# Atif-Anwer/SHMGAN

Hardware: AMD Instinct MI355X
Metric: images/sec (gen+disc train_step) (higher is better)
Workload: dtype f32; 1 GPU; SHMGAN train_step 256x256 5-view, batch 8/GPU, filter_size 64, fp32 (BASELINE configs[1]); global_batch=8, image_size=256, parallelism=dp1, losses_finite=True

## Files before the change

include/shmgan_hip.h:

```cpp
#ifndef SHMGAN_HIP_H
#define SHMGAN_HIP_H

#include <stddef.h>

#ifdef __cplusplus
extern "C" {
#endif

#define SHM_OK 0
#define SHM_E_SHAPE (-1)
#define SHM_E_DTYPE (-2)
#define SHM_E_WORKSPACE (-3)
#define SHM_E_HIP (-4)

#define SHM_F32 0
#define SHM_BF16 1
#define SHM_BF16_GF32 2

int shm_version(void);
const char* shm_last_error(void);
const char* shm_last_kernel(void);

#define SHM_TG_AUTO 0
#define SHM_TG_HALO128 1
#define SHM_TG_HALO64 2
#define SHM_TG_DMA_128x128 3
#define SHM_TG_DMA_64x128 4
#define SHM_TG_DMA_128x64 5
#define SHM_TG_DMA_256x64 6
#define SHM_TG_DMA_256x128 7
#define SHM_TG_HALO128_PH8 8
#define SHM_TG_DMA_128x128_BK32 9
#define SHM_TG_DMA_128x128_NST4 10
#define SHM_TG_HALO128_ST 12
#define SHM_TG_HALO64_ST 13
#define SHM_TG_PHASE4 14
#define SHM_TG_DMA_64x64 15
#define SHM_TG_HALO128_ST_W4 16
#define SHM_TG_WREG 11
int shm_set_tuning(const char* key, int value);
int shm_get_tuning(const char* key, int* value);

int shm_transpose_taps(const float* w, void* wt, int ntaps, int rows, int cols, int rows_pad,
                       int dtype, void* stream);
int shm_transpose_taps_multi(int count, const void* const* w, void* const* wt, const int* ntaps, const int* rows,
                             const int* cols, const int* rows_pad, int dtype, void* stream);
int shm_cast_f32(const float* src, void* dst, size_t n, int dtype, void* stream);

int shm_conv2d_fwd(const void* x, const void* x2, int c1, int ldx, int ldx2, const void* wk,
                   const float* bias, void* y, int ldy, int batch, int hi, int wi, int cin,
                   int cout, int ksize, int stride, float slope, int dtype, void* stream);

#define SHM_STATS_SLOTS 16
int shm_conv2d_in_fwd(const void* x, const void* x2, int c1, int ldx, int ldx2, const void* wk,
                      const float* bias, void* y, int ldy, int batch, int hi, int wi, int cin,
                      int cout, int ksize, int stride, float slope, double* stats, double* scratch,
                      float eps, int dtype, void* stream);

int shm_conv2d_dgrad(const void* dy, int lddy, const void* w, void* dx, void* dx2, int n1,
                     int lddx, int lddx2, int batch, int hi, int wi, int cin, int cout,
                     int ksize, int stride, int dtype, void* stream);

int shm_conv2d_transpose_fwd(const void* x, int ldx, const void* w, const float* bias, void* y,
                             int ldy, int batch, int hi, int wi, int cin, int cout, float slope,
                             int dtype, void* stream);

size_t shm_conv2d_wgrad_workspace(int batch, int ho, int wo, int cin, int cout, int ksize);
int shm_conv2d_wgrad_partial(const void* x, const void* x2, int c1, int ldx, int ldx2, const void* dy,
                             int lddy, int batch, int hi, int wi, int cin, int cin_ld, int cout,
                             int ksize, int stride, void* workspace, size_t ws_bytes, int dtype,
                             int* nsplit_out, void* stream);
// ... 209 lines not shown
```

shmgan_amd/csrc/common.h:

```cpp
#pragma once
#include <hip/hip_runtime.h>
#include <stddef.h>
#include <stdint.h>
#include <stdio.h>

#include "../../include/shmgan_hip.h"

typedef float f32x4 __attribute__((ext_vector_type(4)));
typedef float f32x16 __attribute__((ext_vector_type(16)));

typedef __bf16 bf16_t;

void shm_set_error(const char* fmt, ...);
void shm_set_last_kernel(const char* fmt, ...);

int shm_rgb_s2_fwd_launch(const void* x, int ldx, const void* wk, int K, const float* bias, void* y, int ldy, int batch, int hi, int wi, int cout, float slope,
                          double* stats, int stats_slots, unsigned stats_stride, size_t xbytes, size_t ybytes, int dtype, hipStream_t st);
int shm_rgb_s2_wgrad_launch(const void* x, int ldx, const void* dy, int lddy, float* part, size_t ws_bytes, int batch, int hi, int wi, int cin, int cout,
                            size_t xbytes, size_t dybytes, int dtype, int* nsplit_out, hipStream_t st);

int shm_in_finalize_internal(double* stats, double* part, int nslot, int total, int hw, double eps, float* nt, const float* beta, int c, hipStream_t st);
int shm_gsum_reduce_internal(const void* g, int ldg, const void* aux, int ldaux, double* red, int batch, int hw, int c, int dtype, hipStream_t st);

enum ShmTune {
    SHM_TUNE_TAPGEMM_VARIANT = 0,
    SHM_TUNE_TAPGEMM_HALO_MIN,
    SHM_TUNE_TAPGEMM_SMALL_GRID,
    SHM_TUNE_TAPGEMM_PHASE4_MIN,
    SHM_TUNE_WGRAD_VARIANT,
    SHM_TUNE_WGRAD_BLOCKS,
    SHM_TUNE_WGRAD_BF16_ROWS,
    SHM_TUNE_STATS_FUSION,
    SHM_TUNE_ELEM_REVERSE,
    SHM_TUNE_ELEM_REDUCE_BLOCKS,
    SHM_TUNE_ELEM_NT,
    SHM_TUNE_ELEM_CHUNK_MB,
    SHM_TUNE_ELEM_INTERLEAVE,
    SHM_TUNE_ELEM_STREAM_BLOCKS,
    SHM_TUNE_ELEM_APPLY_BLOCKS,
    SHM_TUNE_TAPGEMM_WREG16,
    SHM_TUNE_WGRAD_BF16_WIDE,
    SHM_TUNE_WGRAD_F32_SPLIT,
    SHM_TUNE_TAPGEMM_FLAT_EPILOGUE,
    SHM_TUNE_ELEM_FUSED_BWD,
    SHM_TUNE_ELEM_FUSED_MAX_SLICES,
    SHM_TUNE_CONV_F32_SPLIT,
    SHM_TUNE_ELEM_FUSED_TEST_STALL,
    SHM_TUNE_ELEM_FUSED_HOLD,
    SHM_TUNE_ELEM_FUSED_GVARIANT,
    SHM_TUNE_COUNT
};
int shm_tune(int id);
unsigned long long* shm_clock_probe();

#define SHM_LDS_BARRIER()                                       \
    do {                                                        \
        asm volatile("s_waitcnt lgkmcnt(0)" ::: "memory");      \
        __builtin_amdgcn_s_barrier();                           \
    } while (0)

typedef unsigned shm_u32x4 __attribute__((ext_vector_type(4)));
__device__ __forceinline__ shm_u32x4 shm_rsrc_words(const void* p, unsigned bytes) {
    const unsigned long long a = (unsigned long long)p;
    return shm_u32x4{(unsigned)a, (unsigned)(a >> 32) & 0xffffu, bytes, 0x00020000u};
}
__device__ __forceinline__ void shm_dma16(const shm_u32x4 rs, const unsigned lds_addr, const unsigned voff) {
    unsigned keep;
    asm volatile("s_mov_b32 %0, m0\n\ts_mov_b32 m0, %1\n\ts_nop 0\n\tbuffer_load_dwordx4 %2, %3, 0 offen lds\n\ts_mov_b32 m0, %0"
                 : "=&s"(keep)
                 : "s"(lds_addr), "v"(voff), "s"(rs)
                 : "memory");
}
__device__ __forceinline__ unsigned shm_lds_addr(const void* p) {
    return (unsigned)(size_t)(__attribute__((address_space(3))) const void*)p;
}

#define SHM_TG_COUNT 17

__device__ __forceinline__ f32x4 ld4(const float* p) { return *(const f32x4*)p; }
__device__ __forceinline__ f32x4 ld4(const bf16_t* p) {
    const uint2 u = *(const uint2*)p;
    f32x4 r;
    r[0] = __uint_as_float(u.x << 16);
    r[1] = __uint_as_float(u.x & 0xffff0000u);
    r[2] = __uint_as_float(u.y << 16);
    r[3] = __uint_as_float(u.y & 0xffff0000u);
    return r;
}
__device__ __forceinline__ f32x4 ld4nt(const float* p) { return __builtin_nontemporal_load((const f32x4*)p); }
__device__ __forceinline__ f32x4 ld4nt(const bf16_t* p) {
    typedef unsigned u32x2_t __attribute__((ext_vector_type(2)));
    const u32x2_t u = __builtin_nontemporal_load((const u32x2_t*)p);
    f32x4 r;
    r[0] = __uint_as_float(u[0] << 16);
    r[1] = __uint_as_float(u[0] & 0xffff0000u);
    r[2] = __uint_as_float(u[1] << 16);
    r[3] = __uint_as_float(u[1] & 0xffff0000u);
    return r;
}
__device__ __forceinline__ void st4(float* p, f32x4 v) { *(f32x4*)p = v; }
__device__ __forceinline__ void st4(bf16_t* p, f32x4 v) {
    typedef bf16_t bf16x4_t __attribute__((ext_vector_type(4)));
    bf16x4_t o;
    o[0] = (bf16_t)v[0];
    o[1] = (bf16_t)v[1];
    o[2] = (bf16_t)v[2];
    o[3] = (bf16_t)v[3];
    *(bf16x4_t*)p = o;
}
__device__ __forceinline__ float rnd_as(const float*, float v) { return v; }
// ... 111 lines not shown
```

shmgan_amd/csrc/conv_igemm.hip:

```cpp
#include "tapgemm.h"

struct ConvExtras {
    double* stats = nullptr;
    int stats_hw = 0, stats_slots = 1;
    const void* gaux[2] = {};
    int ldgaux[2] = {};
    double* gred[2] = {};
    ShmNormReq norm = {};
    bool gsum_fused = false;
};

static TapGemmPlan tapgemm_plan(const TapGemmArgs& a, int batch, int nphase, int esz, int oesz, bool two_src, bool want_norm) {
    const int BKE = 64 / esz;
    const int forced = shm_tune(SHM_TUNE_TAPGEMM_VARIANT);
    bool halo_ok = nphase == 1 && a.is == 1 && a.os == 1 && a.ph[0].ntaps == 9 && a.hi % 16 == 0 && a.wi % 16 == 0 && a.hg == a.hi && a.wg == a.wi;
    if (halo_ok)
        for (int t = 0; t < 9; ++t)
            halo_ok = halo_ok && a.ph[0].dh[t] >= -1 && a.ph[0].dh[t] <= 1 && a.ph[0].dw[t] >= -1 && a.ph[0].dw[t] <= 1;
    const bool bk32_ok = a.K % (2 * BKE) == 0 && (!two_src || a.c1 % (2 * BKE) == 0);
    const bool wreg_ok = esz == 2 && halo_ok && !two_src && (a.K == 32 || a.K == 64) && a.ybytes != 0 && (a.y2 == nullptr || a.y2bytes != 0) &&
                         a.slope >= 0.f && a.slope <= 1.f &&
                         (oesz == 4 || (a.nout % 64 == 0 && a.n1 % 32 == 0 && a.ldy % 8 == 0 && ((size_t)a.y & 15) == 0 &&
                                        (a.y2 == nullptr || (a.ldy2 % 8 == 0 && ((size_t)a.y2 & 15) == 0))));
    const int wreg32_wn = a.nout % 64 == 0 ? 4 : a.nout == 32 ? 2 : a.nout == 16 ? 1 : 0;
    const bool wreg32_ok = esz == 4 && oesz == 4 && halo_ok && (!two_src || (a.c1 == 16 && a.K == 32 && a.nout == 16)) && a.ybytes != 0 &&
                           (a.y2 == nullptr || a.y2bytes != 0) && a.slope >= 0.f && a.slope <= 1.f && a.n1 % 16 == 0 &&
                           ((wreg32_wn == 4 && (a.K == 16 || a.K == 32 || a.K == 64)) || (wreg32_wn == 2 && a.hi % 16 == 0 && (a.K == 16 || a.K == 32)) ||
                            (wreg32_wn == 1 && a.hi % 32 == 0 && (a.K == 16 || a.K == 32)));
    bool phase4_ok = nphase == 4 && a.is == 1 && a.os == 2 && !two_src && a.y2 == nullptr && a.stats == nullptr && a.hi % 16 == 0 &&
                     a.wi % 16 == 0 && a.hg == a.hi && a.wg == a.wi && a.ho == 2 * a.hi && a.wo == 2 * a.wi && a.nout % 64 == 0 &&
                     a.ph[0].ntaps == 4 && a.ph[1].ntaps == 2 && a.ph[2].ntaps == 2 && a.ph[3].ntaps == 1;
    if (phase4_ok)
        for (int p = 0; p < 4; ++p)
            for (int t = 0; t < a.ph[p].ntaps; ++t)
                phase4_ok = phase4_ok && a.ph[p].dh[t] >= -1 && a.ph[p].dh[t] <= 1 && a.ph[p].dw[t] >= -1 && a.ph[p].dw[t] <= 1;
    int v = forced;
    if (v == SHM_TG_AUTO) {
        const long tiles128 = (long)shm_cdiv(a.M, 128) * shm_cdiv(a.nout, 128) * nphase;
        if (wreg_ok || wreg32_ok) {
            v = SHM_TG_WREG;
        } else if (phase4_ok && (long)batch * (a.hi / 16) * (a.wi / 16) * (a.nout / 64) >= shm_tune(SHM_TUNE_TAPGEMM_PHASE4_MIN) &&
                   (esz == 2 || a.K <= 256)) {
            v = SHM_TG_PHASE4;
        } else if (halo_ok) {
            const long np16 = (long)batch * (a.hi / 16) * (a.wi / 16);
            const long nb128 = np16 * shm_cdiv(a.nout, 128), nb64 = np16 * shm_cdiv(a.nout, 64);
            auto fill = [](long nb) { return (double)nb / (double)(((nb + 511) / 512) * 512); };
            if (esz == 4 && nb64 < 256)
                v = SHM_TG_DMA_64x64;
            else if (a.nout <= 64)
                v = SHM_TG_HALO64_ST;
            else if (esz == 4 && nb128 < shm_tune(SHM_TUNE_TAPGEMM_HALO_MIN))
                v = (double)((nb128 + 255) / 256) <= (double)((nb64 + 255) / 256) * 0.52 ? SHM_TG_HALO128_ST : SHM_TG_HALO64_ST;
            else if (nb128 >= (esz == 2 ? 512 : shm_tune(SHM_TUNE_TAPGEMM_HALO_MIN)) || fill(nb128) * 1.03 >= fill(nb64))
                v = SHM_TG_HALO128_ST;
            else
                v = SHM_TG_HALO64_ST;
        } else if ((long)shm_cdiv(a.M, 64) * shm_cdiv(a.nout, 128) * nphase < 256) {
            v = SHM_TG_DMA_64x64;
        } else if (nphase == 1 && a.nout > 64 && a.K <= (esz == 2 ? 256 : 128) &&
                   (long)shm_cdiv(a.M, 256) * shm_cdiv(a.nout, 128) >= 256) {
            v = SHM_TG_DMA_256x128;
        } else if (nphase == 1 && a.nout > 64 && bk32_ok && (esz == 2 ? a.K >= 256 : (a.K >= 256 && a.K < 512 && a.is == 2 && tiles128 >= 512))) {
            v = SHM_TG_DMA_128x128_BK32;
        } else if (a.nout > 64 && tiles128 < shm_tune(SHM_TUNE_TAPGEMM_SMALL_GRID)) {
            v = SHM_TG_DMA_64x128;
        } else if (a.nout > 64) {
            v = SHM_TG_DMA_128x128;
        } else {
            v = SHM_TG_DMA_128x64;
        }
    }
    const bool want_gs = a.gred[0] || a.gred[1];
    bool gs_fused = false;
    if (want_gs) {
        bool al = true;
        for (int p = 0; p < 2; ++p)
            if (a.gred[p]) al = al && (oesz == 4 || (a.ldgaux[p] % 8 == 0 && ((size_t)a.gaux[p] & 15) == 0));
        al = al && (a.y2 == nullptr || a.n1 % 32 == 0);
        const bool small = a.ybytes != 0 && (a.y2 == nullptr || a.y2bytes != 0);
        const bool wide_ok = oesz == 4 || ((a.nout % 8 == 0) && (a.n1 % 8 == 0) && (a.ldy % 8 == 0) && (((size_t)a.y & 15) == 0) &&
                                           (a.y2 == nullptr || ((a.ldy2 % 8 == 0) && (((size_t)a.y2 & 15) == 0))));
        al = al && wide_ok;
        switch (v) {
        case SHM_TG_HALO128_ST: case SHM_TG_HALO64_ST:
            gs_fused = al && small && (a.y2 == nullptr || a.n1 % 64 == 0);
            break;
        case SHM_TG_DMA_128x128: case SHM_TG_DMA_64x128: case SHM_TG_DMA_128x64: case SHM_TG_DMA_64x64: case SHM_TG_DMA_256x64:
        case SHM_TG_DMA_256x128: case SHM_TG_DMA_128x128_BK32: case SHM_TG_DMA_128x128_NST4:
            gs_fused = al && (a.hg * a.wg) % 64 == 0;
            break;
        case SHM_TG_WREG:
            gs_fused = al && small && ((wreg_ok && oesz == 2) || (wreg32_ok && wreg32_wn == 4 && !two_src));
            break;
        case SHM_TG_PHASE4:
            gs_fused = oesz == 4 && small && a.gred[1] == nullptr;
            break;
        default:
            break;
        }
    }
    bool norm_ok = false;
    if (want_norm) {
        const int pc = a.ntpart ? a.K - a.c1 : a.c1;
        norm_ok = !want_gs && nphase == 1 && a.ntc == pc && pc % BKE == 0 && pc <= SHM_NT_MAXC && (a.ntpart == 0 || two_src);
        switch (v) {
        case SHM_TG_HALO128_ST: case SHM_TG_HALO64_ST:
            norm_ok = norm_ok && halo_ok && oesz == esz;
            break;
        case SHM_TG_WREG:
            norm_ok = norm_ok && a.ntpart == 0 && pc <= 64 && ((wreg_ok && oesz == 2) || (wreg32_ok && wreg32_wn == 4 && !two_src));
            break;
        default:
            norm_ok = false;
        }
    }
    const bool x3 = esz == 4 && oesz == 4 && shm_tune(SHM_TUNE_CONV_F32_SPLIT) == 1 && halo_ok && (!want_norm || a.ntmode == 0) &&
                    (v == SHM_TG_HALO128_ST || v == SHM_TG_HALO64_ST || (v == SHM_TG_WREG && forced == SHM_TG_AUTO)) && (!want_gs || gs_fused) && shm_x3_fwd_eligible(a);
    const int w16 = shm_tune(SHM_TUNE_TAPGEMM_WREG16);
    int wreg16 = 0;
    if (v == SHM_TG_WREG && wreg_ok && oesz == 2 && w16 != 0 && !gs_fused && !want_norm && a.nout % 64 == 0 && (a.y2 == nullptr || a.n1 % 64 == 0) && !two_src &&
        a.ybytes != 0 && (a.y2 == nullptr || a.y2bytes != 0))
        wreg16 = w16 == 2 && shm_pp_eligible(a) ? 2 : 1;
    return TapGemmPlan{v, gs_fused, norm_ok, halo_ok, bk32_ok, wreg_ok, wreg32_ok, phase4_ok, wreg32_wn, x3, wreg16};
}

static int finish_args(TapGemmArgs& a, int batch, int nphase, int dtype, bool two_src, const char* who, const ConvExtras& ex) {
    SHM_REQUIRE(dtype == SHM_F32 || dtype == SHM_BF16 || dtype == SHM_BF16_GF32, SHM_E_DTYPE,
                "%s: dtype %d not in {SHM_F32, SHM_BF16, SHM_BF16_GF32}", who, dtype);
    a.stats = ex.stats;
    a.hw = ex.stats_hw;
    a.stats_slots = ex.stats_slots;
    a.stats_stride = (unsigned)batch * (unsigned)a.nout * 2u;
    for (int p = 0; p < 2; ++p) {
        a.gaux[p] = ex.gaux[p];
        a.ldgaux[p] = ex.ldgaux[p];
        a.gred[p] = ex.gred[p];
    }
    a.gslots = SHM_GSUM_SLOTS;
    a.gbatch = batch;
    a.nt = ex.norm.nt;
    a.ntpart = ex.norm.part;
    a.ntc = ex.norm.c;
    a.ntmode = ex.norm.mode;
    a.ntbytes = (unsigned)((size_t)batch * SHM_NT_PLANES * ex.norm.c * sizeof(float));
    a.wimg = 0;
    a.bias_img = 0;
    if (a.gred[0] || a.gred[1]) {
        SHM_REQUIRE(a.stats == nullptr, SHM_E_SHAPE, "%s: fused forward statistics and gsum are exclusive", who);
        a.hw = a.hg * a.wg;
    }
    SHM_REQUIRE(dtype != SHM_BF16_GF32 || a.stats == nullptr, SHM_E_DTYPE, "%s: SHM_BF16_GF32 has no fused statistics", who);
    const int esz = dtype == SHM_F32 ? 4 : 2, bke = 64 / esz, che = 16 / esz;
    SHM_REQUIRE(a.K % bke == 0 && a.K > 0, SHM_E_SHAPE, "%s: contraction channels %d must be a multiple of %d", who, a.K, bke);
    SHM_REQUIRE(a.c1 % bke == 0, SHM_E_SHAPE, "%s: concat split %d must be a multiple of %d", who, a.c1, bke);
    SHM_REQUIRE(a.ldx % che == 0 && (!two_src || a.ldx2 % che == 0), SHM_E_SHAPE, "%s: input pitch must be a multiple of 16 bytes", who);
    SHM_REQUIRE((size_t)batch * a.hi * a.wi < (1u << 31) && (size_t)batch * a.ho * a.wo < (1u << 31), SHM_E_SHAPE, "%s: pixel count overflows int32", who);
// ... 11 lines not shown
        if (a.nt && a.ntmode) {
            SHM_REQUIRE(nphase == 1 && a.bias, SHM_E_SHAPE, "%s: SHM_NORM_SCALED takes per-sample weights AND per-sample bias rows", who);
            a.wimg = (unsigned)((size_t)a.ph[0].ntaps * a.nout * a.K * esz);
            a.bias_img = a.nout;
            wb = (size_t)batch * a.wimg;
        }
        SHM_REQUIRE(xb < lim && x2b < lim && wb < lim, SHM_E_SHAPE, "%s: operand larger than 4 GiB (32-bit buffer offsets)", who);
        a.xbytes = (unsigned)xb;
        a.x2bytes = (unsigned)x2b;
        a.wbytes = (unsigned)wb;
        const int oesz = dtype == SHM_BF16 ? 2 : 4;
        const size_t yb = (size_t)batch * a.ho * a.wo * a.ldy * oesz, y2b = a.y2 ? (size_t)batch * a.ho * a.wo * a.ldy2 * oesz : 0;
        const bool flat = shm_tune(SHM_TUNE_TAPGEMM_FLAT_EPILOGUE) != 0;
        a.ybytes = (yb < lim && !flat) ? (unsigned)yb : 0u;
        a.y2bytes = (y2b < lim && !flat) ? (unsigned)y2b : 0u;
    }
    return SHM_OK;
}

static int device_cus() {
    static const int ncu = [] {
        int dev = 0, n = 0;
        if (hipGetDevice(&dev) != hipSuccess || hipDeviceGetAttribute(&n, hipDeviceAttributeMultiprocessorCount, dev) != hipSuccess || n <= 0) n = 256;
        return n;
    }();
    return ncu;
}

static int launch_plan(const TapGemmArgs& a, const TapGemmPlan& p, int batch, int nphase, int dtype, hipStream_t st, const char* who) {
    if (p.x3) return shm_x3_fwd_launch(a, batch, p.gs_fused, st, who);
    switch (p.variant) {
    case SHM_TG_HALO128: case SHM_TG_HALO64: case SHM_TG_HALO128_ST: case SHM_TG_HALO128_ST_W4: case SHM_TG_HALO64_ST: case SHM_TG_HALO128_PH8:
        return shm_halo_launch(a, p, batch, dtype, st, who);
    case SHM_TG_PHASE4:
        return shm_phase4_launch(a, p, batch, dtype, st, who);
    case SHM_TG_WREG: {
        SHM_REQUIRE(p.wreg_ok || p.wreg32_ok, SHM_E_SHAPE,
                    "%s: forced variant wreg needs a unit-stride 3x3 layer on a map that is a multiple of 16, slope in [0,1] and: bf16 -- one source "
                    "tensor with 32/64 channels, Cout %% 64 == 0; fp32 -- one source with 16/32/64 input channels and "
                    "Cout %% 64 == 0, or 16/32 input channels with Cout = 32 (map a multiple of 16) or 16 (map a multiple of 32; also 16 + 16 from two tensors)", who);
        const int np8 = batch * (a.hi / 8) * (a.wi / 16), ncu = device_cus();
        if (p.wreg16 == 2) return shm_pp_launch(a, batch, ncu, st, who);
        if (p.wreg16 == 1) return shm_wreg16_launch(a, np8, ncu, st, who);
        return p.wreg_ok ? shm_wreg_launch(a, p, np8, ncu, dtype, st, who) : shm_wreg_f32_launch(a, p, batch, ncu, st, who);
    }
    case SHM_TG_DMA_128x128: case SHM_TG_DMA_64x128: case SHM_TG_DMA_128x64: case SHM_TG_DMA_64x64: case SHM_TG_DMA_256x64:
    case SHM_TG_DMA_256x128: case SHM_TG_DMA_128x128_BK32: case SHM_TG_DMA_128x128_NST4:
        return shm_dma_launch(a, p, nphase, dtype, st, who);
    default:
        SHM_REQUIRE(false, SHM_E_SHAPE, "%s: unknown tapgemm.variant %d", who, p.variant);
    }
    return SHM_OK;
}

static int launch_tapgemm(TapGemmArgs& a, int batch, int nphase, int dtype, hipStream_t st, const char* who, ConvExtras& ex) {
    const bool two_src = a.x2 != nullptr;
    if (const int r = finish_args(a, batch, nphase, dtype, two_src, who, ex)) return r;
    if (a.M == 0 || a.nout == 0) return SHM_OK;
    const int esz = dtype == SHM_F32 ? 4 : 2, oesz = dtype == SHM_BF16 ? 2 : 4;
    if (nphase == 1 && a.is == 2 && a.os == 1 && a.ph[0].ntaps == 9 && a.ph[0].dh[0] == 0 && a.ph[0].dw[0] == 0 && !a.x2 && !a.y2 && !a.gred[0] && !a.gred[1] &&
        !a.nt && a.ldx * esz == 16 && a.K * esz == 64 && a.ybytes != 0 && dtype != SHM_BF16_GF32 &&
        shm_tune(SHM_TUNE_TAPGEMM_VARIANT) == SHM_TG_AUTO) {
        const int r = shm_rgb_s2_fwd_launch(a.x, a.ldx, a.w, a.K, a.bias, a.y, a.ldy, batch, a.hi, a.wi, a.nout, a.slope, a.stats, a.stats_slots, a.stats_stride,
                                            a.xbytes, a.ybytes, dtype, st);
        if (r < 0) return r;
        if (r == 1) return SHM_OK;
    }
    const TapGemmPlan p = tapgemm_plan(a, batch, nphase, esz, oesz, two_src, a.nt != nullptr);
// ... 391 lines not shown
```

shmgan_amd/csrc/conv_phase4.hip:

```cpp
#include "tapgemm_dev.h"

template <typename T, typename TO>
__global__ __launch_bounds__(512, 2) void tapgemm_phase4_kernel(const TapGemmArgs a) {
    constexpr int ESZ = sizeof(T), CHE = 16 / ESZ, BKE = 64 / ESZ;
    constexpr int HC = 18, NIT = 24, NHR = NIT * 16;
    constexpr int ASTG = NHR * 16, BTAP = 64 * 16, BSTG = 9 * BTAP;
    extern __shared__ __attribute__((aligned(1024))) float psm[];
    float* const sA = psm;
    float* const sB = psm + 2 * ASTG;
    typedef __attribute__((address_space(3))) void* lds_ptr;

    const int tid = threadIdx.x;
    const int lane = tid & 63, wave = __builtin_amdgcn_readfirstlane(tid >> 6);
    const int l31 = lane & 31, h = lane >> 5;
    const int wm = wave >> 1, wn = wave & 1;
    const int ppr = a.wi >> 4, ppi = (a.hi >> 4) * ppr;
    const int img = blockIdx.x / ppi, prem = blockIdx.x - img * ppi;
    const int y0 = (prem / ppr) << 4, x0 = (prem % ppr) << 4;
    const int n0 = blockIdx.y * 64;

    const int drow = lane >> 2, dq = lane & 3;
    unsigned arow[3];
#pragma unroll
    for (int j = 0; j < 3; ++j) {
        const int hrow = 16 * (wave + 8 * j) + drow;
        const int hr = hrow / HC, hc = hrow - hr * HC;
        const int iy = y0 - 1 + hr, ix = x0 - 1 + hc;
        const bool v = hrow < HC * HC && (unsigned)iy < (unsigned)a.hi && (unsigned)ix < (unsigned)a.wi;
        const int pix = (img * a.hi + iy) * a.wi + ix;
        arow[j] = v ? (unsigned)(pix * a.ldx + (dq ^ (((hrow >> 1) + hr) & 3)) * CHE) * (unsigned)ESZ : 0xffffffffu;
    }
    unsigned wrow[5];
#pragma unroll
// ... 163 lines not shown
                const unsigned ao = pix0 * ldab + nlb, yo = pix0 * ldyb + nyb;
                float q[16];
#pragma unroll
                for (int r = 0; r < 16; ++r) {
                    if constexpr (sizeof(T) == 4)
                        q[r] = __builtin_bit_cast(float, __builtin_amdgcn_raw_buffer_load_b32(rsa, ao, row_pix(r) * ldab, 0));
                    else
                        q[r] = __uint_as_float((unsigned)__builtin_amdgcn_raw_buffer_load_b16(rsa, ao, row_pix(r) * ldab, 0) << 16);
                }
                if (ncol < a.nout) {
#pragma unroll
                    for (int r = 0; r < 16; ++r) {
                        const TO vo = (TO)shm_lrelu(acc[p][i][0][r] + bcol, a.slope);
                        const float v = (float)vo;
                        s1 += v;
                        s2 += v * q[r];
                        if constexpr (sizeof(TO) == 4)
                            __builtin_amdgcn_raw_buffer_store_b32(__builtin_bit_cast(unsigned, vo), rsy, yo, row_pix(r) * ldyb, 0);
                        else
                            __builtin_amdgcn_raw_buffer_store_b16(__builtin_bit_cast(unsigned short, vo), rsy, yo, row_pix(r) * ldyb, 0);
                    }
                }
            }
        const float t1 = s1 + __shfl_xor(s1, 32, 64), t2 = s2 + __shfl_xor(s2, 32, 64);
        if (h == 0 && ncol < a.nout) {
            const int slot = (prem * 4 + wm) % a.gslots;
            double* dst = a.gred[0] + ((size_t)slot * a.gbatch * a.nout + (size_t)img * a.nout + ncol) * 2;
            atomicAdd(dst, (double)t1);
            atomicAdd(dst + 1, (double)t2);
        }
    }
}

template <typename T, typename TO>
static int phase4_launch_t(const TapGemmArgs& a, int batch, hipStream_t st, const char* who) {
    constexpr unsigned kLds = (2 * 24 * 16 * 16 + 2 * 9 * 64 * 16) * sizeof(float);
    static const hipError_t attr = hipFuncSetAttribute((const void*)tapgemm_phase4_kernel<T, TO>, hipFuncAttributeMaxDynamicSharedMemorySize, kLds);
    SHM_REQUIRE(attr == hipSuccess, SHM_E_HIP, "%s: cannot reserve 120 KiB of LDS: %s", who, hipGetErrorString(attr));
    hipLaunchKernelGGL((tapgemm_phase4_kernel<T, TO>), dim3(batch * (a.hi / 16) * (a.wi / 16), a.nout / 64, 1), dim3(512), kLds, st, a);
    shm_set_last_kernel("tapgemm_phase4_kernel<%s, %s>", shm_tg_name<T>(), shm_tg_name<TO>());
    return SHM_OK;
}

int shm_phase4_launch(const TapGemmArgs& a, const TapGemmPlan& p, int batch, int dtype, hipStream_t st, const char* who) {
    SHM_REQUIRE(p.phase4_ok, SHM_E_SHAPE,
                "%s: forced variant phase4 needs a four-phase stride-2 transposed 3x3 product on a 16-aligned input map, one source and one "
                "destination tensor, Cout %% 64 == 0, no fused statistics", who);
    int rc = SHM_OK;
    SHM_DISPATCH_G(dtype, who, rc = phase4_launch_t<T, TG>(a, batch, st, who));
    return rc;
}
```

shmgan_amd/csrc/runtime.hip:

```cpp
#include "common.h"

#include <stdarg.h>

static thread_local char g_err[512] = "";

void shm_set_error(const char* fmt, ...) {
    va_list ap;
    va_start(ap, fmt);
    vsnprintf(g_err, sizeof(g_err), fmt, ap);
    va_end(ap);
}

static thread_local char g_kernel[128] = "";

void shm_set_last_kernel(const char* fmt, ...) {
    va_list ap;
    va_start(ap, fmt);
    vsnprintf(g_kernel, sizeof(g_kernel), fmt, ap);
    va_end(ap);
}

#include <atomic>
#include <stdlib.h>
#include <string.h>
namespace {
struct TuneDef {
    const char* key;
    const char* env;
    int dflt, lo, hi;
};
const TuneDef kTune[SHM_TUNE_COUNT] = {
    {"tapgemm.variant", "SHM_TAPGEMM_VARIANT", 0, 0, SHM_TG_COUNT - 1},
    {"tapgemm.halo_min_blocks", "SHM_TAPGEMM_HALO_MIN", 1024, 0, 1 << 30},
    {"tapgemm.small_grid_blocks", "SHM_TAPGEMM_SMALLM", 1024, 0, 1 << 30},
    {"tapgemm.phase4_min_blocks", "SHM_TAPGEMM_PHASE4_MIN", 256, 0, 1 << 30},
    {"wgrad.variant", "SHM_WGRAD_VARIANT", 0, 0, 3},
    {"wgrad.blocks", "SHM_WGRAD_BLOCKS", 0, 0, 1 << 20},
    {"wgrad.bf16_rows", "SHM_WGRAD_BF16_ROWS", 0, 0, 4},
    {"stats.fusion", "SHM_STATS_FUSION", 1, 0, 1},
    {"elem.reverse", "SHM_ELEM_REVERSE", 1, 0, 1},
    {"elem.reduce_blocks", "SHM_ELEM_REDUCE_BLOCKS", 0, 0, 1 << 20},
    {"elem.nt_loads", "SHM_ELEM_NT", 0, 0, 1},
    {"elem.chunk_mb", "SHM_ELEM_CHUNK_MB", 0, 0, 1 << 20},
    {"elem.interleave", "SHM_ELEM_INTERLEAVE", 1, 0, 1},
    {"elem.stream_blocks", "SHM_ELEM_STREAM_BLOCKS", 32768, 256, 1 << 20},
    {"elem.apply_blocks", "SHM_ELEM_APPLY_BLOCKS", 4096, 256, 1 << 20},
    {"tapgemm.wreg16", "SHM_TAPGEMM_WREG16", 2, 0, 2},
    {"wgrad.bf16_wide", "SHM_WGRAD_BF16_WIDE", 0, 0, 4},
    {"wgrad.f32_split", "SHM_WGRAD_F32_SPLIT", 0, 0, 1},
    {"tapgemm.flat_epilogue", "SHM_TAPGEMM_FLAT_EPILOGUE", 0, 0, 1},
    {"elem.fused_bwd", "SHM_ELEM_FUSED_BWD", 1, 0, 1},
    {"elem.fused_max_slices", "SHM_ELEM_FUSED_MAX_SLICES", 256, 1, 512},
    {"conv.f32_split", "SHM_CONV_F32_SPLIT", 0, 0, 1},
    {"elem.fused_test_stall", "SHM_ELEM_FUSED_TEST_STALL", 0, 0, 1},
    {"elem.fused_hold", "SHM_ELEM_FUSED_HOLD", 0, 0, 2},
    {"elem.fused_gvariant", "SHM_ELEM_FUSED_GVARIANT", 0, 0, 1},
};
std::atomic<int> g_tune[SHM_TUNE_COUNT];
std::atomic<int> g_tune_init{0};
void tune_init() {
    if (g_tune_init.load(std::memory_order_acquire) == 2) return;
    int expect = 0;
    if (g_tune_init.compare_exchange_strong(expect, 1)) {
        for (int i = 0; i < SHM_TUNE_COUNT; ++i) {
            const char* e = getenv(kTune[i].env);
            int v = e ? atoi(e) : kTune[i].dflt;
            if (v < kTune[i].lo || v > kTune[i].hi) v = kTune[i].dflt;
            g_tune[i].store(v);
        }
        g_tune_init.store(2, std::memory_order_release);
    } else {
        while (g_tune_init.load(std::memory_order_acquire) != 2) {
        }
    }
}
int tune_find(const char* key) {
    if (!key) return -1;
    for (int i = 0; i < SHM_TUNE_COUNT; ++i)
        if (strcmp(key, kTune[i].key) == 0) return i;
    return -1;
}
}

int shm_tune(int id) {
    tune_init();
    return g_tune[id].load(std::memory_order_relaxed);
}

extern "C" int shm_set_tuning(const char* key, int value) {
// ... 33 lines not shown
```

shmgan_amd/csrc/tapgemm.h:

```cpp
#pragma once
#include "common.h"
#include "ablate.h"

typedef unsigned u32x4 __attribute__((ext_vector_type(4)));

struct TapPhase {
    int oph, opw, ntaps;
    int dh[9], dw[9], widx[9];
};

typedef __bf16 bf16x8 __attribute__((ext_vector_type(8)));
typedef __bf16 bf16x2_t __attribute__((ext_vector_type(2)));
typedef float f32x2 __attribute__((ext_vector_type(2)));
typedef short s16x4_t __attribute__((ext_vector_type(4)));
typedef __attribute__((address_space(3))) s16x4_t* lds_s16x4_t;

struct TapGemmArgs {
    const void* x;
    const void* x2;
    int c1, ldx, ldx2;
    const void* w;
    const float* bias;
    void* y;
    void* y2;
    int n1, ldy, ldy2;
    int hi, wi, K;
    int hg, wg;
    int ho, wo, nout;
    int is, os;
    int M;
    unsigned xbytes, x2bytes, wbytes;
    unsigned ybytes, y2bytes;
    double* stats;
    int hw;
    int stats_slots;
    unsigned stats_stride;
    float slope;
    const void* gaux[2];
    int ldgaux[2];
    double* gred[2];
    int gslots, gbatch;
    const float* nt;
    int ntpart, ntc, ntmode;
    unsigned ntbytes, wimg;
    int bias_img;
    TapPhase ph[4];
};

struct TapGemmPlan {
    int variant;
    bool gs_fused, norm_ok;
    bool halo_ok, bk32_ok, wreg_ok, wreg32_ok, phase4_ok;
    int wreg32_wn;
    bool x3;
    int wreg16;
};

template <typename T>
constexpr const char* shm_tg_name() { return sizeof(T) == 4 ? "float" : "__bf16"; }

int shm_dma_launch(const TapGemmArgs& a, const TapGemmPlan& p, int nphase, int dtype, hipStream_t st, const char* who);
int shm_halo_launch(const TapGemmArgs& a, const TapGemmPlan& p, int batch, int dtype, hipStream_t st, const char* who);
int shm_phase4_launch(const TapGemmArgs& a, const TapGemmPlan& p, int batch, int dtype, hipStream_t st, const char* who);
int shm_wreg_launch(const TapGemmArgs& a, const TapGemmPlan& p, int np8, int ncu, int dtype, hipStream_t st, const char* who);
int shm_wreg_f32_launch(const TapGemmArgs& a, const TapGemmPlan& p, int batch, int ncu, hipStream_t st, const char* who);

int shm_wreg16_launch(const TapGemmArgs& a, int np8, int ncu, hipStream_t st, const char* who);

int shm_x3_fwd_eligible(const TapGemmArgs& a);
int shm_x3_fwd_launch(const TapGemmArgs& a, int batch, bool gs_fused, hipStream_t st, const char* who);

int shm_pp_eligible(const TapGemmArgs& a);
int shm_pp_launch(const TapGemmArgs& a, int batch, int ncu, hipStream_t st, const char* who);
```

shmgan_amd/ops.py:

```python
from __future__ import annotations

import torch

from ._lib import check, lib


def _stream():
    return torch.cuda.current_stream().cuda_stream


class KernelTimer:

    def __init__(self):
        self.recs = []
        self.brecs = []

    def wrap(self, sym, flops, fn, label="", fixed=False):
        e0 = torch.cuda.Event(enable_timing=True)
        e1 = torch.cuda.Event(enable_timing=True)
        e0.record()
        fn()
        e1.record()
        if not fixed:
            k = lib().shm_last_kernel()
# ... 47 lines not shown
    else:
        TIMER.wrap(sym, flops, fn, label)


def _timed_bytes(name, nbytes, fn):
    if TIMER is None:
        fn()
    else:
        TIMER.wrap_bytes(name, nbytes, fn)


def _p(t):
    return 0 if t is None else t.data_ptr()


def _dt(t):
    if t.dtype == torch.bfloat16:
        return 1
    if t.dtype == torch.float32:
        return 0
    raise TypeError(f"activation tensors are float32 or bfloat16, got {t.dtype}")


def _dtg(act, grad):
    d = _dt(act)
    if d == 1 and grad is not None and grad.dtype == torch.float32:
        return 2
    if grad is not None and d != 2 and _dt(grad) != d:
        raise TypeError("gradient-signal tensors are float32, or share the activation dtype")
    return d


TAPGEMM_VARIANTS = {"auto": 0, "halo128": 1, "halo64": 2, "dma128x128": 3, "dma64x128": 4, "dma128x64": 5, "dma256x64": 6,
                    "dma256x128": 7, "halo128_ph8": 8, "dma128x128_bk32": 9, "dma128x128_nst4": 10, "wreg": 11, "halo128_st": 12, "halo64_st": 13, "phase4": 14, "dma64x64": 15, "halo128_st_w4": 16}


def set_tuning(key, value):
    if isinstance(value, str):
        value = TAPGEMM_VARIANTS[value]
    check(lib().shm_set_tuning(key.encode(), int(value)), "shm_set_tuning")


def get_tuning(key):
    import ctypes
    v = ctypes.c_int(0)
    check(lib().shm_get_tuning(key.encode(), ctypes.addressof(v)), "shm_get_tuning")
    return v.value


def last_kernel():
    k = lib().shm_last_kernel()
    return k.decode() if k else ""


def cast_f32(src, dst, n):
    check(lib().shm_cast_f32(_p(src), _p(dst), n, _dt(dst), _stream()), "shm_cast_f32")


class TransposeBatch:

    def __init__(self, items):
        import ctypes as C
        self.items = list(items)
        n = len(self.items)
        assert n <= 48
        self.n = n
        self.dt = _dt(self.items[0][1]) if n else 0
# ... 728 lines not shown
```

Before: 69.97 images/sec.

## Add persistent 32-channel phase4 transposed-conv kernel with wave-quantization-aware selection

Adds a persistent-grid variant of the four-phase stride-2 transposed 3x3 kernel for fp32 that works on 32-channel output slices with 256-thread blocks. Each block loops over patches and prefetches the next tile's halo while storing the current results. The auto planner picks it when the 32-wide grid fills the GPU better than the 64-wide one, or when K is large. This targets tail-wave underutilization and per-block launch overhead in the fp32 generator upsampling layers. The cost is a second, smaller-tile code path that reuses less data per block, plus new grid and delay tuning knobs.

```diff
diff --git a/include/shmgan_hip.h b/include/shmgan_hip.h
--- a/include/shmgan_hip.h
+++ b/include/shmgan_hip.h
@@ -37,6 +37,7 @@
 #define SHM_TG_PHASE4 14
 #define SHM_TG_DMA_64x64 15
 #define SHM_TG_HALO128_ST_W4 16
+#define SHM_TG_PHASE4_N32 17
 #define SHM_TG_WREG 11
 int shm_set_tuning(const char* key, int value);
 int shm_get_tuning(const char* key, int* value);
diff --git a/shmgan_amd/csrc/common.h b/shmgan_amd/csrc/common.h
--- a/shmgan_amd/csrc/common.h
+++ b/shmgan_amd/csrc/common.h
@@ -48,6 +48,8 @@
     SHM_TUNE_ELEM_FUSED_TEST_STALL,
     SHM_TUNE_ELEM_FUSED_HOLD,
     SHM_TUNE_ELEM_FUSED_GVARIANT,
+    SHM_TUNE_TAPGEMM_PHASE4_GRID,
+    SHM_TUNE_TAPGEMM_PHASE4_DELAY,
     SHM_TUNE_COUNT
 };
 int shm_tune(int id);
@@ -75,7 +77,7 @@
     return (unsigned)(size_t)(__attribute__((address_space(3))) const void*)p;
 }
 
-#define SHM_TG_COUNT 17
+#define SHM_TG_COUNT 18
 
 __device__ __forceinline__ f32x4 ld4(const float* p) { return *(const f32x4*)p; }
 __device__ __forceinline__ f32x4 ld4(const bf16_t* p) {
diff --git a/shmgan_amd/csrc/conv_igemm.hip b/shmgan_amd/csrc/conv_igemm.hip
--- a/shmgan_amd/csrc/conv_igemm.hip
+++ b/shmgan_amd/csrc/conv_igemm.hip
@@ -34,13 +34,19 @@
         for (int p = 0; p < 4; ++p)
             for (int t = 0; t < a.ph[p].ntaps; ++t)
                 phase4_ok = phase4_ok && a.ph[p].dh[t] >= -1 && a.ph[p].dh[t] <= 1 && a.ph[p].dw[t] >= -1 && a.ph[p].dw[t] <= 1;
+    const bool phase4_n32_ok = phase4_ok && esz == 4 && oesz == 4 && a.ybytes != 0;
+    const long p4_blocks = phase4_ok ? (long)batch * (a.hi / 16) * (a.wi / 16) * (a.nout / 64) : 0;
+    const double p4_fill64 = phase4_ok ? (double)p4_blocks / (double)(((p4_blocks + 255) / 256) * 256) : 0.;
+    const double p4_fill32 = phase4_ok ? (double)(2 * p4_blocks) / (double)(((2 * p4_blocks + 255) / 256) * 256) : 0.;
     int v = forced;
     if (v == SHM_TG_AUTO) {
         const long tiles128 = (long)shm_cdiv(a.M, 128) * shm_cdiv(a.nout, 128) * nphase;
         if (wreg_ok || wreg32_ok) {
             v = SHM_TG_WREG;
-        } else if (phase4_ok && (long)batch * (a.hi / 16) * (a.wi / 16) * (a.nout / 64) >= shm_tune(SHM_TUNE_TAPGEMM_PHASE4_MIN) &&
-                   (esz == 2 || a.K <= 256)) {
+        } else if (phase4_n32_ok && p4_blocks >= shm_tune(SHM_TUNE_TAPGEMM_PHASE4_MIN) && p4_fill32 >= 0.9 &&
+                   (a.K > 256 || p4_fill64 < 0.9 || 2 * p4_blocks >= 3 * 512)) {
+            v = SHM_TG_PHASE4_N32;
+        } else if (phase4_ok && p4_blocks >= shm_tune(SHM_TUNE_TAPGEMM_PHASE4_MIN) && (esz == 2 || a.K <= 256)) {
             v = SHM_TG_PHASE4;
         } else if (halo_ok) {
             const long np16 = (long)batch * (a.hi / 16) * (a.wi / 16);
@@ -93,7 +99,7 @@
         case SHM_TG_WREG:
             gs_fused = al && small && ((wreg_ok && oesz == 2) || (wreg32_ok && wreg32_wn == 4 && !two_src));
             break;
-        case SHM_TG_PHASE4:
+        case SHM_TG_PHASE4: case SHM_TG_PHASE4_N32:
             gs_fused = oesz == 4 && small && a.gred[1] == nullptr;
             break;
         default:
@@ -122,7 +128,7 @@
     if (v == SHM_TG_WREG && wreg_ok && oesz == 2 && w16 != 0 && !gs_fused && !want_norm && a.nout % 64 == 0 && (a.y2 == nullptr || a.n1 % 64 == 0) && !two_src &&
         a.ybytes != 0 && (a.y2 == nullptr || a.y2bytes != 0))
         wreg16 = w16 == 2 && shm_pp_eligible(a) ? 2 : 1;
-    return TapGemmPlan{v, gs_fused, norm_ok, halo_ok, bk32_ok, wreg_ok, wreg32_ok, phase4_ok, wreg32_wn, x3, wreg16};
+    return TapGemmPlan{v, gs_fused, norm_ok, halo_ok, bk32_ok, wreg_ok, wreg32_ok, phase4_ok, phase4_n32_ok, wreg32_wn, x3, wreg16};
 }
 
 static int finish_args(TapGemmArgs& a, int batch, int nphase, int dtype, bool two_src, const char* who, const ConvExtras& ex) {
@@ -200,8 +206,8 @@
     switch (p.variant) {
     case SHM_TG_HALO128: case SHM_TG_HALO64: case SHM_TG_HALO128_ST: case SHM_TG_HALO128_ST_W4: case SHM_TG_HALO64_ST: case SHM_TG_HALO128_PH8:
         return shm_halo_launch(a, p, batch, dtype, st, who);
-    case SHM_TG_PHASE4:
-        return shm_phase4_launch(a, p, batch, dtype, st, who);
+    case SHM_TG_PHASE4: case SHM_TG_PHASE4_N32:
+        return shm_phase4_launch(a, p, batch, device_cus(), dtype, st, who);
     case SHM_TG_WREG: {
         SHM_REQUIRE(p.wreg_ok || p.wreg32_ok, SHM_E_SHAPE,
                     "%s: forced variant wreg needs a unit-stride 3x3 layer on a map that is a multiple of 16, slope in [0,1] and: bf16 -- one source "
diff --git a/shmgan_amd/csrc/conv_phase4.hip b/shmgan_amd/csrc/conv_phase4.hip
--- a/shmgan_amd/csrc/conv_phase4.hip
+++ b/shmgan_amd/csrc/conv_phase4.hip
@@ -1,4 +1,5 @@
 #include "tapgemm_dev.h"
+#include <algorithm>
 
 template <typename T, typename TO>
 __global__ __launch_bounds__(512, 2) void tapgemm_phase4_kernel(const TapGemmArgs a) {
@@ -228,6 +229,245 @@
     }
 }
 
+template <typename T, typename TO, int NB, bool GS>
+__global__ __launch_bounds__(256, 2) void tapgemm_phase4_kernel(const TapGemmArgs a, const int delay) {
+    static_assert(NB == 32 && sizeof(TO) == 4, "the persistent form: 32-channel slices, four-byte outputs");
+    constexpr int ESZ = sizeof(T), CHE = 16 / ESZ, BKE = 64 / ESZ;
+    constexpr int HC = 18, NIT = 21, NHR = NIT * 16;
+    constexpr int ASTG = NHR * 16, BTAP = NB * 16, BSTG = 9 * BTAP;
+    constexpr int NWI = 9 * NB / 16;
+    extern __shared__ __attribute__((aligned(1024))) float psm[];
+    float* const sA = psm;
+    float* const sB = psm + 2 * ASTG;
+    typedef __attribute__((address_space(3))) void* lds_ptr;
+
+    const int tid = threadIdx.x;
+    const int lane = tid & 63, wave = __builtin_amdgcn_readfirstlane(tid >> 6);
+    const int l31 = lane & 31, h = lane >> 5;
+    const int wm = wave;
+    const int ppr = a.wi >> 4, ppi = (a.hi >> 4) * ppr;
+    const int np = a.M >> 8, nsl = a.nout / NB;
+    const int nx = ((gridDim.x | (unsigned)np) & 7) == 0 ? 8 : 1;
+    const int xg = blockIdx.x & (nx - 1), qstep = gridDim.x / nx;
+    int q = blockIdx.x / nx;
+
+    const int drow = lane >> 2, dq = lane & 3;
+    unsigned wrow[5];
+#pragma unroll
+    for (int j = 0; j < 5; ++j) {
+        const int item = wave + 4 * j;
+        const int step = item >> 1;
+        const int ph = step < 4 ? 0 : step < 6 ? 1 : step < 8 ? 2 : 3;
+        const int tp = step < 4 ? step : step < 6 ? step - 4 : step < 8 ? step - 6 : 0;
+        const int row = (item & 1) * 16 + drow;
+        const int wi_ = item < NWI ? a.ph[ph].widx[tp] : 0;
+        wrow[j] = (unsigned)((wi_ * a.nout + row) * a.K + (dq ^ ((row >> 2) & 3)) * CHE) * (unsigned)ESZ;
+    }
+    const __amdgpu_buffer_rsrc_t rsx = __builtin_amdgcn_make_buffer_rsrc((void*)a.x, 0, a.xbytes, 0x00020000);
+    const __amdgpu_buffer_rsrc_t rsw = __builtin_amdgcn_make_buffer_rsrc((void*)a.w, 0, a.wbytes, 0x00020000);
+    const int nch = a.K / BKE;
+
+    unsigned arow[6];
+    auto halo_rows = [&](int img, int y0, int x0) {
+#pragma unroll
+        for (int j = 0; j < 6; ++j) {
+            const int hrow = 16 * (wave + 4 * j) + drow;
+            const int hr = hrow / HC, hc = hrow - hr * HC;
+            const int iy = y0 - 1 + hr, ix = x0 - 1 + hc;
+            const bool v = hrow < HC * HC && (unsigned)iy < (unsigned)a.hi && (unsigned)ix < (unsigned)a.wi;
+            const int pix = (img * a.hi + iy) * a.wi + ix;
+            arow[j] = v ? (unsigned)(pix * a.ldx + (dq ^ (((hrow >> 1) + hr) & 3)) * CHE) * (unsigned)ESZ : 0xffffffffu;
+        }
+    };
+    auto dma = [&](int chunk, int stg, int n0) {
+        const unsigned cb = (unsigned)(chunk * BKE) * (unsigned)ESZ;
+        const unsigned wb = cb + (unsigned)(n0 * a.K) * (unsigned)ESZ;
+        float* da = sA + stg * ASTG + wave * 256;
+        float* db = sB + stg * BSTG + wave * 256;
+#pragma unroll
+        for (int j = 0; j < 6; ++j) {
+            if (j < 5 || wave < 1) {
+                const unsigned off = arow[j] == 0xffffffffu ? arow[j] : arow[j] + cb;
+                __builtin_amdgcn_raw_ptr_buffer_load_lds(rsx, (lds_ptr)(da + j * 4 * 256), 16, (int)off, 0, 0, 0);
+            }
+        }
+#pragma unroll
+        for (int j = 0; j < 5; ++j) {
+            if (j < 4 || wave < 2) {
+                __builtin_amdgcn_raw_ptr_buffer_load_lds(rsw, (lds_ptr)(db + j * 4 * 256), 16, (int)(wrow[j] + wb), 0, 0, 0);
+            }
+        }
+    };
+
+    f32x16 acc[4][2][1];
+#pragma unroll
+    for (int p = 0; p < 4; ++p)
+#pragma unroll
+        for (int i = 0; i < 2; ++i)
+#pragma unroll
+            for (int r = 0; r < 16; ++r) acc[p][i][0][r] = 0.f;
+
+    constexpr int kTile1 = 2 * HC * 16;
+    int fs[9];
+    {
+        const int hb = (4 * wm + (l31 >> 4) + 1) * HC + (l31 & 15) + 1;
+#pragma unroll
+        for (int st = 0; st < 9; ++st) {
+            const int ph = st < 4 ? 0 : st < 6 ? 1 : st < 8 ? 2 : 3;
+            const int tp = st < 4 ? st : st < 6 ? st - 4 : st < 8 ? st - 6 : 0;
+            const int hrow = hb + a.ph[ph].dh[tp] * HC + a.ph[ph].dw[tp];
+            fs[st] = hrow * 16 + ((h ^ (((hrow >> 1) + hrow / HC) & 3)) << 2);
+        }
+    }
+    const int swb = (l31 >> 2) & 3;
+    const int fb0 = l31 * 16 + ((0 + h) ^ swb) * 4, fb1 = l31 * 16 + ((2 + h) ^ swb) * 4;
+    typedef const __attribute__((address_space(3))) f32x4* lds_f4;
+    const unsigned sA_lds = (unsigned)(size_t)(__attribute__((address_space(3))) float*)sA;
+
+    const __amdgpu_buffer_rsrc_t rsy = __builtin_amdgcn_make_buffer_rsrc(a.y, 0, a.ybytes, 0x00020000);
+    const unsigned ldyb = (unsigned)a.ldy * (unsigned)sizeof(TO);
+    auto row_pix = [&](int r) { return (unsigned)(2 * (r >> 3) * a.wo + 16 * ((r >> 2) & 1) + 2 * (r & 3)); };
+
+    int patch = (q / nsl) * nx + xg;
+    if (patch >= np) return;
+    int img = patch / ppi, prem = patch - img * ppi;
+    int y0 = (prem / ppr) << 4, x0 = (prem % ppr) << 4, n0 = (q % nsl) * NB;
+    int stg = 0;
+    float bcol = 0.f;
+    bool stores_behind = false;
+    halo_rows(img, y0, x0);
+    dma(0, 0, n0);
+    if (delay > 0 && (__builtin_amdgcn_s_getreg((3 << 11) | (16 << 6) | 4) & 1u))
+        for (int i = 0; i < delay; ++i) __builtin_amdgcn_s_sleep(127);
+    unsigned stamps[12] = {};
+    int nstamp = 0;
+    auto stamp = [&](int k) {
+        if constexpr (abl::stamp)
+            if (nstamp < 4) stamps[3 * nstamp + k] = (unsigned)__builtin_amdgcn_s_memtime();
+    };
+    for (;;) {
+        stamp(0);
+        for (int chunk = 0; chunk < nch; ++chunk) {
+            if (chunk == 0 && stores_behind)
+                asm volatile("s_waitcnt vmcnt(63)" ::: "memory");
+            else
+                asm volatile("s_waitcnt vmcnt(0)" ::: "memory");
+            SHM_LDS_BARRIER();
+            asm volatile("" ::: "memory");
+            if (chunk + 1 < nch) dma(chunk + 1, stg ^ 1, n0);
+            if (chunk == 0 && a.bias) bcol = a.bias[n0 + l31];
+            const unsigned Ab = sA_lds + (unsigned)(stg * ASTG * 4);
+            const float* Bb = sB + stg * BSTG;
+#pragma unroll
+            for (int st = 0; st < 9; ++st) {
+                constexpr int kPhase[9] = {0, 0, 0, 0, 1, 1, 2, 2, 3};
+#pragma unroll
+                for (int kk = 0; kk < 2; ++kk) {
+                    f32x4 av[2], bv[1];
+#pragma unroll
+                    for (int i = 0; i < 2; ++i)
+                        av[i] = *(lds_f4)(size_t)(((Ab + (unsigned)(fs[st] << 2)) ^ (unsigned)(kk << 5)) + (unsigned)(i * kTile1 * 4));
+                    bv[0] = *(const f32x4*)(Bb + st * BTAP + (kk ? fb1 : fb0));
+                    tap_mfma<T, 2, 1>(av, bv, acc[kPhase[st]]);
+                }
+            }
+            asm volatile("" ::: "memory");
+            stg ^= 1;
+        }
+
+        asm volatile("" : "+v"(bcol));
+        const int cimg = img, cprem = prem, cy0 = y0, cx0 = x0, cn0 = n0;
+        q += qstep;
+        patch = (q / nsl) * nx + xg;
+        const bool more = patch < np;
+        if (more) {
+            img = patch / ppi;
+            prem = patch - img * ppi;
+            y0 = (prem / ppr) << 4;
+            x0 = (prem % ppr) << 4;
+            n0 = (q % nsl) * NB;
+            halo_rows(img, y0, x0);
+            dma(0, stg, n0);
+        }
+        if constexpr (abl::stamp) asm volatile("" ::"v"(acc[3][1][0]));
+        stamp(1);
+
+        const int ncol = cn0 + l31;
+        const unsigned nyb = (unsigned)ncol * (unsigned)sizeof(TO);
+        auto lane_pix0 = [&](int p, int i) {
+            return (unsigned)((cimg * a.ho + (2 * (cy0 + 4 * wm + 2 * i) + a.ph[p].oph)) * a.wo + (2 * (cx0 + 4 * h) + a.ph[p].opw));
+        };
+        if constexpr (!GS) {
+#pragma unroll
+            for (int p = 0; p < 4; ++p)
+#pragma unroll
+                for (int i = 0; i < 2; ++i) {
+                    const unsigned yo = lane_pix0(p, i) * ldyb + nyb;
+#pragma unroll
+                    for (int r = 0; r < 16; ++r) {
+                        const TO vo = (TO)shm_lrelu(acc[p][i][0][r] + bcol, a.slope);
+                        __builtin_amdgcn_raw_buffer_store_b32(__builtin_bit_cast(unsigned, vo), rsy, yo, row_pix(r) * ldyb, 0);
+                    }
+                }
+        } else {
+            const __amdgpu_buffer_rsrc_t rsa = __builtin_amdgcn_make_buffer_rsrc((void*)a.gaux[0], 0, 0xfffffff0u, 0x00020000);
+            const unsigned ldab = (unsigned)a.ldgaux[0] * (unsigned)sizeof(T), nlb = (unsigned)ncol * (unsigned)sizeof(T);
+            float s1 = 0.f, s2 = 0.f;
+#pragma unroll
+            for (int p = 0; p < 4; ++p)
+#pragma unroll
+                for (int i = 0; i < 2; ++i) {
+                    const unsigned pix0 = lane_pix0(p, i);
+                    const unsigned ao = pix0 * ldab + nlb, yo = pix0 * ldyb + nyb;
+                    float qv[16];
+#pragma unroll
+                    for (int r = 0; r < 16; ++r) {
+                        if constexpr (sizeof(T) == 4)
+                            qv[r] = __builtin_bit_cast(float, __builtin_amdgcn_raw_buffer_load_b32(rsa, ao, row_pix(r) * ldab, 0));
+                        else
+                            qv[r] = __uint_as_float((unsigned)__builtin_amdgcn_raw_buffer_load_b16(rsa, ao, row_pix(r) * ldab, 0) << 16);
+                    }
+#pragma unroll
+                    for (int r = 0; r < 16; ++r) {
+                        const TO vo = (TO)shm_lrelu(acc[p][i][0][r] + bcol, a.slope);
+                        const float v = (float)vo;
+                        s1 += v;
+                        s2 += v * qv[r];
+                        __builtin_amdgcn_raw_buffer_store_b32(__builtin_bit_cast(unsigned, vo), rsy, yo, row_pix(r) * ldyb, 0);
+                    }
+                }
+            const float t1 = s1 + __shfl_xor(s1, 32, 64), t2 = s2 + __shfl_xor(s2, 32, 64);
+            if (h == 0) {
+                const int slot = (cprem * 4 + wm) % a.gslots;
+                double* dst = a.gred[0] + ((size_t)slot * a.gbatch * a.nout + (size_t)cimg * a.nout + ncol) * 2;
+                atomicAdd(dst, (double)t1);
+                atomicAdd(dst + 1, (double)t2);
+            }
+        }
+        stamp(2);
+        ++nstamp;
+        if (!more) break;
+        stores_behind = true;
+#pragma unroll
+        for (int p = 0; p < 4; ++p)
+#pragma unroll
+            for (int i = 0; i < 2; ++i)
+#pragma unroll
+                for (int r = 0; r < 16; ++r) acc[p][i][0][r] = 0.f;
+    }
+    if constexpr (abl::stamp) {
+        if (tid == 0 && a.bias) {
+            unsigned* d = (unsigned*)a.bias + a.nout + 16 * blockIdx.x;
+            d[0] = __builtin_amdgcn_s_getreg((31 << 11) | 4);
+            d[1] = __builtin_amdgcn_s_getreg((31 << 11) | 20);
+            d[2] = (unsigned)nstamp;
+            d[3] = 0;
+#pragma unroll
+            for (int k = 0; k < 12; ++k) d[4 + k] = stamps[k];
+        }
+    }
+}
+
 template <typename T, typename TO>
 static int phase4_launch_t(const TapGemmArgs& a, int batch, hipStream_t st, const char* who) {
     constexpr unsigned kLds = (2 * 24 * 16 * 16 + 2 * 9 * 64 * 16) * sizeof(float);
@@ -238,7 +478,26 @@
     return SHM_OK;
 }
 
-int shm_phase4_launch(const TapGemmArgs& a, const TapGemmPlan& p, int batch, int dtype, hipStream_t st, const char* who) {
+template <bool GS>
+static int phase4_n32_launch(const TapGemmArgs& a, int ncu, hipStream_t st, const char* who) {
+    constexpr unsigned kLds = (2 * 21 * 16 * 16 + 2 * 9 * 32 * 16) * sizeof(float);
+    static const hipError_t attr = hipFuncSetAttribute((const void*)tapgemm_phase4_kernel<float, float, 32, GS>, hipFuncAttributeMaxDynamicSharedMemorySize, kLds);
+    SHM_REQUIRE(attr == hipSuccess, SHM_E_HIP, "%s: cannot reserve 78 KiB of LDS: %s", who, hipGetErrorString(attr));
+    const long items = (long)(a.M / 256) * (a.nout / 32);
+    const int want = shm_tune(SHM_TUNE_TAPGEMM_PHASE4_GRID);
+    const long grid = std::min<long>(want > 0 ? want : 2L * ncu, items);
+    const int delay = shm_tune(SHM_TUNE_TAPGEMM_PHASE4_DELAY);
+    hipLaunchKernelGGL((tapgemm_phase4_kernel<float, float, 32, GS>), dim3((unsigned)grid, 1, 1), dim3(256), kLds, st, a, delay);
+    shm_set_last_kernel("tapgemm_phase4_kernel<float, float, 32, %s>", GS ? "true" : "false");
+    return SHM_OK;
+}
+
+int shm_phase4_launch(const TapGemmArgs& a, const TapGemmPlan& p, int batch, int ncu, int dtype, hipStream_t st, const char* who) {
+    if (p.variant == SHM_TG_PHASE4_N32) {
+        SHM_REQUIRE(p.phase4_n32_ok, SHM_E_SHAPE,
+                    "%s: forced variant phase4_n32 needs a shape the variant phase4 takes, fp32 operands and an fp32 output below 4 GiB", who);
+        return a.gred[0] ? phase4_n32_launch<true>(a, ncu, st, who) : phase4_n32_launch<false>(a, ncu, st, who);
+    }
     SHM_REQUIRE(p.phase4_ok, SHM_E_SHAPE,
                 "%s: forced variant phase4 needs a four-phase stride-2 transposed 3x3 product on a 16-aligned input map, one source and one "
                 "destination tensor, Cout %% 64 == 0, no fused statistics", who);
diff --git a/shmgan_amd/csrc/runtime.hip b/shmgan_amd/csrc/runtime.hip
--- a/shmgan_amd/csrc/runtime.hip
+++ b/shmgan_amd/csrc/runtime.hip
@@ -55,6 +55,8 @@
     {"elem.fused_test_stall", "SHM_ELEM_FUSED_TEST_STALL", 0, 0, 1},
     {"elem.fused_hold", "SHM_ELEM_FUSED_HOLD", 0, 0, 2},
     {"elem.fused_gvariant", "SHM_ELEM_FUSED_GVARIANT", 0, 0, 1},
+    {"tapgemm.phase4_grid", "SHM_TAPGEMM_PHASE4_GRID", 0, 0, 1 << 20},
+    {"tapgemm.phase4_delay", "SHM_TAPGEMM_PHASE4_DELAY", 0, 0, 64},
 };
 std::atomic<int> g_tune[SHM_TUNE_COUNT];
 std::atomic<int> g_tune_init{0};
diff --git a/shmgan_amd/csrc/tapgemm.h b/shmgan_amd/csrc/tapgemm.h
--- a/shmgan_amd/csrc/tapgemm.h
+++ b/shmgan_amd/csrc/tapgemm.h
@@ -51,6 +51,7 @@
     int variant;
     bool gs_fused, norm_ok;
     bool halo_ok, bk32_ok, wreg_ok, wreg32_ok, phase4_ok;
+    bool phase4_n32_ok;
     int wreg32_wn;
     bool x3;
     int wreg16;
@@ -61,7 +62,7 @@
 
 int shm_dma_launch(const TapGemmArgs& a, const TapGemmPlan& p, int nphase, int dtype, hipStream_t st, const char* who);
 int shm_halo_launch(const TapGemmArgs& a, const TapGemmPlan& p, int batch, int dtype, hipStream_t st, const char* who);
-int shm_phase4_launch(const TapGemmArgs& a, const TapGemmPlan& p, int batch, int dtype, hipStream_t st, const char* who);
+int shm_phase4_launch(const TapGemmArgs& a, const TapGemmPlan& p, int batch, int ncu, int dtype, hipStream_t st, const char* who);
 int shm_wreg_launch(const TapGemmArgs& a, const TapGemmPlan& p, int np8, int ncu, int dtype, hipStream_t st, const char* who);
 int shm_wreg_f32_launch(const TapGemmArgs& a, const TapGemmPlan& p, int batch, int ncu, hipStream_t st, const char* who);
 
diff --git a/shmgan_amd/ops.py b/shmgan_amd/ops.py
--- a/shmgan_amd/ops.py
+++ b/shmgan_amd/ops.py
@@ -103,7 +103,7 @@
 
 
 TAPGEMM_VARIANTS = {"auto": 0, "halo128": 1, "halo64": 2, "dma128x128": 3, "dma64x128": 4, "dma128x64": 5, "dma256x64": 6,
-                    "dma256x128": 7, "halo128_ph8": 8, "dma128x128_bk32": 9, "dma128x128_nst4": 10, "wreg": 11, "halo128_st": 12, "halo64_st": 13, "phase4": 14, "dma64x64": 15, "halo128_st_w4": 16}
+                    "dma256x128": 7, "halo128_ph8": 8, "dma128x128_bk32": 9, "dma128x128_nst4": 10, "wreg": 11, "halo128_st": 12, "halo64_st": 13, "phase4": 14, "dma64x64": 15, "halo128_st_w4": 16, "phase4_n32": 17}
 
 
 def set_tuning(key, value):
```

Result: no change. 70.38 images/sec, median of 6 (+0.6%).
